# makezur/super_primitive

Hardware: AMD Instinct MI355X
Metric: GN iters/sec (640x480x64-seg frame pairs) (higher is better)
Workload: dtype f32; 1 GPU; Replica-shaped two-frame SfM, 640x480, 64 segments (grid, 4 px overlap), pyramid level 0 of a 3-level pyramid; BASELINE.json configs[1]; pairs_per_gpu=384, segment_pixels_per_pair=373056, optimiser=gn, tile_points=8192, span_points=4096, granule=64

## Files before the change

### super_primitive_amd/csrc/sp_cost.hip

```cpp
#include <type_traits>

#include "sp_solve_device.h"

namespace {

struct TileCtx {
    gptr_u32 pix;
    gptr_f4 src4;
    gptr_f32 trg;
    Cam Ks;
    Warp w;
    float shift;
    float gain, bias;
    float ax, ay;
    uint32_t row_bytes;
    int Wl, Hl;
    int start, count;
};

struct Geo {
    float qx, qy, qz;
    float zinv, zi;
    float px, py, pz;
};
// ... 251 lines not shown
    f32x2 wxy; float m;
    f32x2 srg; float sb;
    uint32_t off0;
};

__device__ __forceinline__ void prepare2_at(const PairConsts& k, f32x2 colrow, bool src_ok, float d, const f32x4 s, Pending2& p);

template <bool DT = false>
__device__ __forceinline__ void prepare2(const TileCtx& c, const PairConsts& k, float shift, uint32_t pw, const f32x4 s, Pending2& p) {
    const f32x2 colrow{(float)(pw & 0xffffu), (float)((pw >> 16) & 0x7fffu)};
    const bool src_ok = (int32_t)pw < 0;
    const float d = DT ? s.w * shift : fast_exp(s.w + shift);
    prepare2_at(k, colrow, src_ok, d, s, p);
}

typedef const SpRunDesc __attribute__((address_space(4)))* cptr_rd;
__device__ __forceinline__ SpRunDesc rd_load(cptr_rd p) {
    SpRunDesc r;
    r.valid[0] = p->valid[0]; r.valid[1] = p->valid[1];
    r.d[0] = p->d[0]; r.d[1] = p->d[1];
    r.base[0] = p->base[0]; r.base[1] = p->base[1];
    r.k = p->k; r.runs = p->runs;
    return r;
}
__device__ __forceinline__ f32x2 rd_colrow(const SpRunDesc& r, f32x2 lane2) {
    const float step = __builtin_amdgcn_fmed3f(lane2.x + r.k, 0.f, 1.f);
    return pfma(step, f32x2{r.d[0], r.d[1]}, lane2) + f32x2{r.base[0], r.base[1]};
}
__device__ __forceinline__ float rd_depth(const SpRunDesc& r, float d) {
    const uint64_t m = ((uint64_t)r.valid[1] << 32) | r.valid[0];
    float o;
    asm("v_cndmask_b32_e64 %0, 0, %1, %2" : "=v"(o) : "v"(d), "s"(m));
    return o;
}
template <bool DT>
__device__ __forceinline__ void prepare2_rd(const PairConsts& k, float shift, const SpRunDesc& r, f32x2 lane2, const f32x4 s, Pending2& p) {
    const f32x2 colrow = rd_colrow(r, lane2);
    const float d = rd_depth(r, DT ? s.w * shift : fast_exp(s.w + shift));
    prepare2_at(k, colrow, true, d, s, p);
}
template <bool DT>
__device__ __forceinline__ void prepare_rd(const TileCtx& c, float shift, float ifx, float ify, const SpRunDesc& r, f32x2 lane2, const f32x4 s,
                                           Pending& p) {
    const f32x2 colrow = rd_colrow(r, lane2);
    const float d = rd_depth(r, DT ? s.w * shift : fast_exp(s.w + shift));
    float x, y;
    backproject(colrow.x, colrow.y, d, c.Ks, ifx, ify, x, y);
    prepare_xyz(c, x, y, d, true, s.x, s.y, s.z, p);
}

__device__ __forceinline__ void prepare2_at(const PairConsts& k, f32x2 colrow, bool src_ok, float d, const f32x4 s, Pending2& p) {
    const f32x2 xy = pfma(colrow, k.ifxy, k.nKc) * d;
    const f32x2 qxy = pfma(k.R03, f32x2{xy.x, xy.x}, pfma(k.R14, f32x2{xy.y, xy.y}, pfma(k.R25, f32x2{d, d}, k.t01)));
    const float qz = fmaf(k.R6, xy.x, fmaf(k.R7, xy.y, fmaf(k.R8, d, k.t2)));
    const bool zguard = fabsf(qz) > 1e-6f;
    const float zinv = zguard ? __builtin_amdgcn_rcpf(qz) : 1e-6f;
    const f32x2 uv = qxy * k.Kf * zinv + k.Ktc;
    const f32x2 n = pfma(uv, k.invWH, f32x2{-1.f, -1.f});
    const bool ok = (fabsf(n.x) <= 0.99f) && (fabsf(n.y) <= 0.99f) && (qz > k.zmin) && src_ok && (d > 1e-7f);
    p.m = ok ? 1.f : 0.f;
    p.qxy = qxy; p.qz = qz;
    p.zinv = ok ? zinv : 0.f;
    p.zi = (ok && zguard) ? zinv : 0.f;
    p.srg = f32x2{s.x, s.y}; p.sb = s.z;
    const f32x2 ixy = pfma(n, k.sxy, k.sxy);
    const f32x2 fl{floorf(ixy.x), floorf(ixy.y)};
    p.wxy = ixy - fl;
    p.off0 = (uint32_t)fmaf(fl.y, k.row_bytes_f, fl.x * (float)(4u * SP_TEXEL_FLOATS));
}

struct Mix2 { f32x2 wa, wb, v; };
struct MixA { f32x2 ua, ub; };
// ... 141 lines not shown
    k.shift = cursor_shift<DT>(k.nq_kld, k.nq_kpl);
    cursor_fetch_next<TRIP>(k);
    return true;
}

template <bool WT>
__device__ __forceinline__ void store_partial(float* p, float v) {
    if (WT) __hip_atomic_store(p, v, __ATOMIC_RELAXED, __HIP_MEMORY_SCOPE_AGENT);
    else *p = v;
}

__device__ __forceinline__ int lane_id() { return (int)__builtin_amdgcn_mbcnt_hi(~0u, __builtin_amdgcn_mbcnt_lo(~0u, 0u)); }

template <bool WT, bool AFF = false>
__device__ __forceinline__ void flush_segment_gn(GnAcc& A, float* __restrict__ rec, AffAcc* aa = nullptr) {
    const int lane = lane_id();
    int pos; bool ok;
    if constexpr (AFF) {
        float v[10] = {A.hd01.x, A.hd01.y, A.hd[0].x, A.hd[0].y, A.hd[1].x, A.hd[1].y, A.D.x + A.D.y, A.bd.x + A.bd.y, aa->hda, aa->hdb};
        wave_sum_to_lanes<10>(v, lane, pos, ok);
        if (ok) store_partial<WT>(rec + pos, v[0]);
        aa->hda = 0.f; aa->hdb = 0.f;
    } else {
        float v[10] = {A.hd01.x, A.hd01.y, A.hd[0].x, A.hd[0].y, A.hd[1].x, A.hd[1].y, A.D.x + A.D.y, A.bd.x + A.bd.y,
                       A.cost - A.cost_mark, A.n - A.n_mark};
        wave_sum_to_lanes<10>(v, lane, pos, ok);
        if (ok) store_partial<WT>(rec + pos, v[0]);
        A.cost_mark = A.cost; A.n_mark = A.n;
    }
    const f32x2 z{0.f, 0.f};
    A.hd01 = z; A.hd[0] = z; A.hd[1] = z; A.D = z; A.bd = z;
}

template <bool DT, bool WT, bool AFF = false, bool W64 = false, bool RD = false>
__device__ __forceinline__ void run_span_gn(const TileCtx& c, const SpPair& pr, const int4* __restrict__ chunks, int q0,
                                            int n_chunks, int total, float irls_eps, float* __restrict__ span_rec,
                                            float* __restrict__ seg_partials, float* lds, const SpRunDesc* rd = nullptr) {
    static_assert(!RD || (W64 && DT && !AFF), "run descriptors: wave spans on depth tables");
    constexpr int TRIP = W64 ? 64 : SP_BLOCK;
    constexpr int NV = AFF ? SP_GNA_PARTIAL_FLOATS : SP_GN_PARTIAL_FLOATS, NS = AFF ? SP_GNA_SEG_FLOATS : SP_GN_SEG_FLOATS;
    GnAcc A;
    AffAcc AA;
    MixA ma{f32x2{0.f, 0.f}, f32x2{0.f, 0.f}};
    {
        const f32x2 z{0.f, 0.f};
        AA.haa = AA.hab = AA.hbb = AA.ba = AA.bb = AA.hda = AA.hdb = 0.f;
        AA.pa01 = z; AA.pb01 = z; AA.pa[0] = z; AA.pa[1] = z; AA.pb[0] = z; AA.pb[1] = z;
    }
    {
        const f32x2 z{0.f, 0.f};
        A.h00 = z; A.bp01 = z; A.hd01 = z;
#pragma unroll
        for (int k = 0; k < 2; ++k) { A.h0[k] = z; A.h1[k] = z; A.bp[k] = z; A.hd[k] = z; }
#pragma unroll
        for (int k = 0; k < 6; ++k) A.blk[k] = z;
        A.D = z; A.bd = z;
        A.h11 = A.cost = A.n = A.cost_mark = A.n_mark = 0.f;
    }
    const int wave = __builtin_amdgcn_readfirstlane((int)(threadIdx.x >> 6));
    SpanCursor k;
    cursor_init<TRIP, DT>(k, pr, chunks, q0, n_chunks);
    const int start = k.chunks[q0].start;
    PairConsts kc;
    {
        const Warp& w = c.w;
        kc.ifxy = sgpr2(1.f / c.Ks.fx, 1.f / c.Ks.fy);
        kc.nKc = f32x2{-c.Ks.cx * (1.f / c.Ks.fx), -c.Ks.cy * (1.f / c.Ks.fy)};
        kc.R03 = sgpr2(w.R[0], w.R[3]);        kc.R14 = sgpr2(w.R[1], w.R[4]);      kc.R25 = sgpr2(w.R[2], w.R[5]);
        kc.t01 = f32x2{w.t[0], w.t[1]};        kc.Kf = sgpr2(w.Kt.fx, w.Kt.fy);     kc.Ktc = sgpr2(w.Kt.cx, w.Kt.cy);
        kc.invWH = sgpr2(2.f * w.invWm1, 2.f * w.invHm1);  kc.sxy = sgpr2(w.sx, w.sy);
        kc.gab = sgpr2(c.gain * c.ax * w.Kt.fx, c.gain * c.ay * w.Kt.fy);
        kc.bias2 = f32x2{c.bias, c.bias};      kc.eps2 = sgpr2(irls_eps, irls_eps);
        kc.R6 = sgpr(w.R[6]); kc.R7 = sgpr(w.R[7]); kc.R8 = sgpr(w.R[8]); kc.t2 = w.t[2];
        asm volatile("" : "+v"(kc.nKc), "+v"(kc.bias2), "+v"(kc.t01), "+v"(kc.t2));
        kc.gain = sgpr(c.gain); kc.bias = sgpr(c.bias); kc.zmin = sgpr(w.zmin); kc.eps = sgpr(irls_eps);
        kc.row_bytes_f = sgpr((float)(c.Wl * (int)(4u * SP_TEXEL_FLOATS)));
    }
    const rsrc_t r_pix = make_rsrc(c.pix + start, (uint32_t)total * 4u);
    const rsrc_t r_src = make_rsrc(c.src4 + start, (uint32_t)total * 16u);
    const rsrc_t r_trg = make_rsrc(c.trg, (uint32_t)c.Wl * (uint32_t)c.Hl * (4u * SP_TEXEL_FLOATS));
    const int n_iter = total / TRIP;
    uint32_t op = (W64 ? (threadIdx.x & 63u) : threadIdx.x) * 4u;
    constexpr int NT = 2;
    cptr_rd rg = (cptr_rd)rd + (start >> 6);
    f32x2 lane2{(float)(threadIdx.x & 63u), 0.f};
    if (RD) asm volatile("" : "+v"(lane2));
    struct Slot { Pending2 p; int q; bool last; };
    Slot S0, S1;
    {
        const f32x4 s = buf_load4<NT>(r_src, op * 4u);
        if (RD) prepare2_rd<DT>(kc, k.shift, rd_load(rg), lane2, s, S0.p);
        else {
            const uint32_t pw = (uint32_t)__builtin_amdgcn_raw_buffer_load_b32(r_pix, (int)op, 0, NT);
            prepare2<DT>(c, kc, k.shift, pw, s, S0.p);
        }
        S0.last = cursor_advance<TRIP, DT>(k, S0.q);
    }
    S1.p = S0.p;
    S1.p.zinv = 0.f; S1.p.zi = 0.f;
    S1.q = q0; S1.last = false;
    Mix2 m{f32x2{0.f, 0.f}, f32x2{0.f, 0.f}, f32x2{0.f, 0.f}};
    auto trip = [&](Slot& a, Slot& b) {
        op += 4u * TRIP;
        asm volatile("" : "+v"(op));
        const uint32_t pw = RD ? 0u : (uint32_t)__builtin_amdgcn_raw_buffer_load_b32(r_pix, (int)op, 0, NT);
        const f32x4 s = buf_load4<NT>(r_src, op * 4u);
        SpRunDesc rn;
        if (RD) { ++rg; rn = rd_load(rg); }
        f32x3 ta = buf_load3(r_trg, a.p.off0);
        f32x3 tb = buf_load3(r_trg, a.p.off0 + 4u * SP_TEXEL_FLOATS);
        f32x3 tc = buf_load3(r_trg, a.p.off0, c.row_bytes);
        f32x3 td = buf_load3(r_trg, a.p.off0 + 4u * SP_TEXEL_FLOATS, c.row_bytes);
        __builtin_amdgcn_sched_barrier(0);
        fold_gn2<AFF>(kc, GeoGn{b.p.qxy, b.p.qz, b.p.zinv, b.p.zi}, m, A, &ma, &AA);
        if (b.last) flush_segment_gn<WT, AFF>(A, seg_partials + (size_t)(W64 ? b.q : 4 * b.q + wave) * NS, &AA);
        __builtin_amdgcn_sched_barrier(0);
        asm volatile("" : "+v"(ta), "+v"(tb), "+v"(tc), "+v"(td), "+v"(A.blk[0]), "+v"(A.blk[1]), "+v"(A.blk[2]),
                     "+v"(A.blk[3]), "+v"(A.blk[4]), "+v"(A.blk[5]), "+v"(A.bp[0]), "+v"(A.bp[1]), "+v"(A.hd[0]),
                     "+v"(A.hd[1]), "+v"(A.D), "+v"(A.bd), "+v"(A.h00), "+v"(A.h0[0]), "+v"(A.h0[1]), "+v"(A.h1[0]), "+v"(A.h1[1]), "+v"(A.h11), "+v"(A.bp01), "+v"(A.hd01));
        finish_gn2<AFF>(kc, a.p, ta, tb, tc, td, m, A.cost, A.n, &ma, &AA);
        uint32_t pw_ = pw;
        f32x4 s_ = s;
        if (RD) asm volatile("" : "+v"(s_));
        else asm volatile("" : "+v"(pw_), "+v"(s_));
        if (RD) prepare2_rd<DT>(kc, k.shift, rn, lane2, s_, b.p);
        else prepare2<DT>(c, kc, k.shift, pw_, s_, b.p);
        b.last = cursor_advance<TRIP, DT>(k, b.q);
    };
    int j = 0;
    for (; j + 1 < n_iter; j += 2) { trip(S0, S1); trip(S1, S0); }
    if (j < n_iter) {
        trip(S0, S1);
        fold_gn2<AFF>(kc, GeoGn{S0.p.qxy, S0.p.qz, S0.p.zinv, S0.p.zi}, m, A, &ma, &AA);
        flush_segment_gn<WT, AFF>(A, seg_partials + (size_t)(W64 ? S0.q : 4 * S0.q + wave) * NS, &AA);
    } else {
        fold_gn2<AFF>(kc, GeoGn{S1.p.qxy, S1.p.qz, S1.p.zinv, S1.p.zi}, m, A, &ma, &AA);
        flush_segment_gn<WT, AFF>(A, seg_partials + (size_t)(W64 ? S1.q : 4 * S1.q + wave) * NS, &AA);
    }
    float acc[NV];
    acc[0] = A.cost;
    acc[1] = A.h00.x; acc[2] = A.h00.y;
    acc[3] = A.h0[0].x; acc[4] = A.h0[0].y; acc[5] = A.h0[1].x; acc[6] = A.h0[1].y;
    acc[7] = A.h11;
    acc[8] = A.h1[0].x; acc[9] = A.h1[0].y; acc[10] = A.h1[1].x; acc[11] = A.h1[1].y;
    acc[12] = A.blk[0].x; acc[13] = A.blk[0].y; acc[14] = A.blk[1].x; acc[15] = A.blk[1].y;
    acc[16] = A.blk[2].y; acc[17] = A.blk[3].x; acc[18] = A.blk[3].y;
    acc[19] = A.blk[4].x; acc[20] = A.blk[4].y; acc[21] = A.blk[5].y;
    acc[22] = A.bp01.x; acc[23] = A.bp01.y;
    acc[24] = A.bp[0].x; acc[25] = A.bp[0].y; acc[26] = A.bp[1].x; acc[27] = A.bp[1].y;
    acc[28] = A.n;
    if constexpr (AFF) {
        acc[29] = AA.haa; acc[30] = AA.hab; acc[31] = AA.hbb; acc[32] = AA.ba; acc[33] = AA.bb;
        acc[34] = AA.pa01.x; acc[35] = AA.pa01.y; acc[36] = AA.pa[0].x; acc[37] = AA.pa[0].y; acc[38] = AA.pa[1].x; acc[39] = AA.pa[1].y;
        acc[40] = AA.pb01.x; acc[41] = AA.pb01.y; acc[42] = AA.pb[0].x; acc[43] = AA.pb[0].y; acc[44] = AA.pb[1].x; acc[45] = AA.pb[1].y;
        acc[46] = acc[47] = 0.f;
    } else {
        acc[29] = acc[30] = acc[31] = 0.f;
    }
    if (W64) {
        int pos; bool ok;
        wave_sum_to_lanes<NV>(acc, (int)((op >> 2) & 63u), pos, ok);
        if (ok) store_partial<WT>(span_rec + pos, acc[0]);
    } else {
        const int tid = (int)((op >> 2) & (uint32_t)(SP_BLOCK - 1));
        const float tot = block_sum_to_thread<NV>(acc, lds, tid);
        if (tid < NV) store_partial<WT>(span_rec + tid, tot);
    }
}

template <bool DT, bool WT, bool W64 = false, bool RD = false>
__device__ __forceinline__ void run_span_grad(const TileCtx& c, const SpPair& pr, const int4* __restrict__ chunks, int q0,
                                              int n_chunks, int total, float* __restrict__ span_rec,
                                              float* __restrict__ seg_partials, float* lds, const SpRunDesc* rd = nullptr) {
    static_assert(!RD || (W64 && DT), "run descriptors: wave spans on depth tables");
    constexpr int TRIP = W64 ? 64 : SP_BLOCK;
    constexpr int NV = SP_GRAD_PARTIAL_FLOATS;
    float acc[NV];
#pragma unroll
    for (int i = 0; i < NV; ++i) acc[i] = 0.f;
    const int wave = __builtin_amdgcn_readfirstlane((int)(threadIdx.x >> 6));
    SpanCursor k;
    cursor_init<TRIP, DT>(k, pr, chunks, q0, n_chunks);
    const int start = k.chunks[q0].start;
    const float ifx = 1.f / c.Ks.fx, ify = 1.f / c.Ks.fy;
    const rsrc_t r_pix = make_rsrc(c.pix + start, (uint32_t)total * 4u);
    const rsrc_t r_src = make_rsrc(c.src4 + start, (uint32_t)total * 16u);
    const rsrc_t r_trg = make_rsrc(c.trg, (uint32_t)c.Wl * (uint32_t)c.Hl * (4u * SP_TEXEL_FLOATS));
    const int n_iter = total / TRIP;
    uint32_t op = (W64 ? (threadIdx.x & 63u) : threadIdx.x) * 4u;
    constexpr int NT = 2;
    cptr_rd rg = (cptr_rd)rd + (start >> 6);
    f32x2 lane2{(float)(threadIdx.x & 63u), 0.f};
    if (RD) asm volatile("" : "+v"(lane2));
    struct Slot { Pending p; int q; bool last; };
    Slot S0, S1;
    {
        const f32x4 s = buf_load4<NT>(r_src, op * 4u);
        if (RD) prepare_rd<DT>(c, k.shift, ifx, ify, rd_load(rg), lane2, s, S0.p);
        else {
            const uint32_t pw = (uint32_t)__builtin_amdgcn_raw_buffer_load_b32(r_pix, (int)op, 0, NT);
// ... 175 lines not shown
    int32_t first_block;
    uint32_t mask;
    int32_t vspans;
};
struct SchedCost {
    const SpPair* pairs[SP_MAX_PHASES];
    float irls_eps[SP_MAX_PHASES];
    uint32_t mask;
    int32_t vspans;
    int32_t n_lists;
    SchedList list[SP_SCHED_LISTS];
};
struct FuseArgs {
    int32_t* arrivals;
    AdamArgs adam;
    GnArgs gn;
    const int32_t* done;
    const int32_t* phase;
    SchedCost sched;
    const int32_t* active;
    const MultiList* multi;
    int32_t n_multi;
    const uint32_t* rd_pix;
    const SpRunDesc* rd_desc;
};

constexpr int FORM_LOG_DEPTH = 0, FORM_DEPTH = 6;

struct Pix;
struct RunDesc;
template <class SRC>
struct CostFrom {
template <int MODE, int FORM = FORM_LOG_DEPTH, int FUSED = 0, bool W64 = false>
static __global__ __launch_bounds__(SP_BLOCK, FUSED != 0 ? 1 : (MODE == 2 ? 2 : 4)) void k_cost_pairs(
        const SpPair* __restrict__ pairs, const int4* __restrict__ chunks, const int4* __restrict__ spans, int n_spans,
        float irls_eps, float* __restrict__ partials, float* __restrict__ seg_partials, FuseArgs f) {
    static_assert(FORM == FORM_LOG_DEPTH || FORM == FORM_DEPTH, "FORM: log-depth tables (0) or depth tables (6)");
    constexpr bool RD = std::is_same<SRC, RunDesc>::value;
    constexpr bool DT = FORM == FORM_DEPTH;
    constexpr int NV = MODE == 0 ? SP_GRAD_PARTIAL_FLOATS : (MODE == 2 ? SP_GNA_PARTIAL_FLOATS : SP_GN_PARTIAL_FLOATS);
    __shared__ float lds[SP_WAVES * NV];
    int block = blockIdx.x;
    uint32_t phase_mask = f.sched.mask;
    int vspans = f.sched.vspans;
    if (f.multi) {
        int l = 0;
        for (int i = 1; i < f.n_multi && block >= f.multi[i].first_block; ++i) l = i;
        const MultiList& ml = f.multi[l];
        block -= ml.first_block;
        pairs = ml.pairs; chunks = reinterpret_cast<const int4*>(ml.chunks); spans = reinterpret_cast<const int4*>(ml.spans);
        n_spans = ml.n_spans; partials = ml.partials; seg_partials = ml.seg_partials;
    }
    if (f.phase && f.sched.n_lists > 0) {
        int l = 0;
#pragma unroll
        for (int i = 1; i < SP_SCHED_LISTS; ++i)
            if (i < f.sched.n_lists && block >= f.sched.list[i].first_block) l = i;
        const SchedList& sl = f.sched.list[l];
        block -= sl.first_block;
        chunks = sl.chunks; spans = sl.spans; n_spans = sl.n_spans; partials = sl.partials; seg_partials = sl.seg_partials;
        phase_mask = sl.mask;
        vspans = sl.vspans;
    }
    int w = W64 ? 4 * xcd_chunked_tile(block, (n_spans + 3) >> 2) + __builtin_amdgcn_readfirstlane((int)(threadIdx.x >> 6))
                : xcd_chunked_tile(block, n_spans);
    if (w >= n_spans) return;
    int owner;
// ... 7 lines not shown
        pairs = f.sched.pairs[ph];
        irls_eps = f.sched.irls_eps[ph];
        if (j >= pairs[owner].n_tiles) return;
        w = pairs[owner].tile0 + j;
        span = spans[w];
    } else {
        span = spans[w];
        owner = span.w;
        if (f.done && f.done[owner]) return;
        if (f.phase) {
            const int ph = f.phase[owner];
            if (ph >= SP_MAX_PHASES || ph < 0 || !((phase_mask >> ph) & 1u)) return;
            pairs = f.sched.pairs[ph];
            irls_eps = f.sched.irls_eps[ph];
        }
    }
    const SpPair& pr = pairs[owner];
    TileCtx c;
    c.pix = (gptr_u32)pr.pix;
    c.src4 = (gptr_f4)pr.src4;
    c.trg = (gptr_f32)pr.trg3;
    c.Ks = Cam{pr.K_src[0], pr.K_src[1], pr.K_src[2], pr.K_src[3]};
    const Cam Kt{pr.K_trg[0], pr.K_trg[1], pr.K_trg[2], pr.K_trg[3]};
    fill_warp(c, pr.pose, Kt, pr.H, pr.W, pr.Hl, pr.Wl, pr.zmin);
    c.shift = 0.f;
    c.gain = 1.f; c.bias = 0.f;
    if (pr.aff) {
        c.gain = sgpr(expf(-(pr.aff[2] - pr.aff[0])));
        c.bias = sgpr(pr.aff[3] - pr.aff[1]);
    }
    c.start = 0; c.count = 0;
    const SpRunDesc* rd = RD ? f.rd_desc + ((const uint32_t*)pr.pix - f.rd_pix) / 64 : nullptr;
    if (MODE == 2) run_span_gn<DT, FUSED != 0, true>(c, pr, chunks, span.x, span.y, span.z, irls_eps, partials + (size_t)w * NV, seg_partials, lds);
    else if (MODE == 1) run_span_gn<DT, FUSED != 0, false, W64, RD>(c, pr, chunks, span.x, span.y, span.z, irls_eps, partials + (size_t)w * NV, seg_partials, lds, rd);
    else run_span_grad<DT, FUSED != 0, W64, RD>(c, pr, chunks, span.x, span.y, span.z, partials + (size_t)w * NV, seg_partials, lds, rd);
    if (FUSED != 0) {
        __shared__ int is_last;
        asm volatile("s_waitcnt vmcnt(0)" ::: "memory");
        __syncthreads();
        if (threadIdx.x == 0) {
            const int old = __hip_atomic_fetch_add(f.arrivals + span.w, 1, __ATOMIC_RELAXED, __HIP_MEMORY_SCOPE_AGENT);
            const int last = old == pr.n_tiles - 1;
            if (last) {
                __hip_atomic_store(f.arrivals + span.w, 0, __ATOMIC_RELAXED, __HIP_MEMORY_SCOPE_AGENT);
                __builtin_amdgcn_fence(__ATOMIC_ACQUIRE, "agent");
            }
            is_last = last;
        }
        __syncthreads();
        if (is_last) {
            if (FUSED == 1) solve_adam(pairs, span.w, partials, seg_partials, f.adam);
            else solve_gn(pairs, span.w, partials, seg_partials, f.gn);
        }
    }
}
};

struct CostVariant {
    int mode;
    bool dt, w64, rd;
    int fused;
};
using CostKernel = void (*)(const SpPair*, const int4*, const int4*, int, float, float*, float*, FuseArgs);
CostKernel cost_kernel(const CostVariant& v) {
    enum { DT = 4, W64 = 8, RD = 16, ADAM = 32, GN = 2 * ADAM };
    if (v.mode < 0 || v.mode > 2 || v.fused < 0 || v.fused > 2) return nullptr;
    switch (v.mode | (v.dt ? DT : 0) | (v.w64 ? W64 : 0) | (v.rd ? RD : 0) | v.fused * ADAM) {
// ... 305 lines not shown
```

Before: 443,100 iters/s.

## Process two pixel groups per lane with packed-math Gauss-Newton span kernel

Adds a new wave-span GN path that handles two 64-pixel groups per lane at once, packing their geometry, residuals and normal-equation accumulation into v_pk_* f32x2 instructions via inline asm. The goal is to raise packed-FMA throughput and expose more memory-level parallelism per wave. It also lowers the occupancy hint for that kernel variant to 2 blocks, since the doubled accumulators raise register pressure. The older W64/run-descriptor code in run_span_gn is removed and routed to the new function instead.

```diff
diff --git a/super_primitive_amd/csrc/sp_cost.hip b/super_primitive_amd/csrc/sp_cost.hip
--- a/super_primitive_amd/csrc/sp_cost.hip
+++ b/super_primitive_amd/csrc/sp_cost.hip
@@ -307,12 +307,6 @@
     float o;
     asm("v_cndmask_b32_e64 %0, 0, %1, %2" : "=v"(o) : "v"(d), "s"(m));
     return o;
-}
-template <bool DT>
-__device__ __forceinline__ void prepare2_rd(const PairConsts& k, float shift, const SpRunDesc& r, f32x2 lane2, const f32x4 s, Pending2& p) {
-    const f32x2 colrow = rd_colrow(r, lane2);
-    const float d = rd_depth(r, DT ? s.w * shift : fast_exp(s.w + shift));
-    prepare2_at(k, colrow, true, d, s, p);
 }
 template <bool DT>
 __device__ __forceinline__ void prepare_rd(const TileCtx& c, float shift, float ifx, float ify, const SpRunDesc& r, f32x2 lane2, const f32x4 s,
@@ -520,12 +514,444 @@
     A.hd01 = z; A.hd[0] = z; A.hd[1] = z; A.D = z; A.bd = z;
 }
 
-template <bool DT, bool WT, bool AFF = false, bool W64 = false, bool RD = false>
+typedef f32x2 P2;
+__device__ __forceinline__ P2 bc(float v) { return P2{v, v}; }
+__device__ __forceinline__ P2 lo2(P2 v) { return P2{v.x, v.x}; }
+__device__ __forceinline__ P2 hi2(P2 v) { return P2{v.y, v.y}; }
+
+struct PendingP {
+    P2 qx, qy, qz, zinv, zi;
+    P2 wx, wy, m;
+    f32x2 srgA, srgB;
+    P2 sb;
+    uint32_t offA, offB;
+};
+struct MixP { P2 w00, w01, w11, v0, v1, t; };
+struct AccP {
+    P2 h00, h01, h11, h0[4], h1[4];
+    P2 blk[10];
+    P2 bp[6];
+    P2 seg[10];
+    float cost, n;
+};
+
+__device__ __forceinline__ P2 psub2_lo(P2 a, f32x2 b) {
+    P2 d;
+    asm("v_pk_add_f32 %0, %1, %2 op_sel_hi:[1,0] neg_lo:[0,1] neg_hi:[0,1]" : "=v"(d) : "v"(a), "v"(b));
+    return d;
+}
+__device__ __forceinline__ P2 psub2_hi(P2 a, f32x2 b) {
+    P2 d;
+    asm("v_pk_add_f32 %0, %1, %2 op_sel:[0,1] op_sel_hi:[1,1] neg_lo:[0,1] neg_hi:[0,1]" : "=v"(d) : "v"(a), "v"(b));
+    return d;
+}
+__device__ __forceinline__ float fma3(float a, float b, float c) {
+    float d;
+    asm("v_fma_f32 %0, %1, %2, %3" : "=v"(d) : "v"(a), "v"(b), "v"(c));
+    return d;
+}
+__device__ __forceinline__ P2 pfma_s_lo(f32x2 s, P2 b, f32x2 c) {
+    P2 d;
+    asm("v_pk_fma_f32 %0, %1, %2, %3 op_sel_hi:[0,1,0]" : "=v"(d) : "s"(s), "v"(b), "v"(c));
+    return d;
+}
+__device__ __forceinline__ P2 pfma_s_hi(f32x2 s, P2 b, f32x2 c) {
+    P2 d;
+    asm("v_pk_fma_f32 %0, %1, %2, %3 op_sel:[1,0,1] op_sel_hi:[1,1,1]" : "=v"(d) : "s"(s), "v"(b), "v"(c));
+    return d;
+}
+__device__ __forceinline__ P2 pmul_b_lo(P2 a, f32x2 B) {
+    P2 d;
+    asm("v_pk_mul_f32 %0, %1, %2 op_sel_hi:[1,0]" : "=v"(d) : "v"(a), "v"(B));
+    return d;
+}
+__device__ __forceinline__ P2 pmul_b_hi(P2 a, f32x2 B) {
+    P2 d;
+    asm("v_pk_mul_f32 %0, %1, %2 op_sel:[0,1] op_sel_hi:[1,1]" : "=v"(d) : "v"(a), "v"(B));
+    return d;
+}
+__device__ __forceinline__ P2 pfma_c_lo(P2 a, P2 b, f32x2 C) {
+    P2 d;
+    asm("v_pk_fma_f32 %0, %1, %2, %3 op_sel_hi:[1,1,0]" : "=v"(d) : "v"(a), "v"(b), "v"(C));
+    return d;
+}
+__device__ __forceinline__ P2 pfma_c_hi(P2 a, P2 b, f32x2 C) {
+    P2 d;
+    asm("v_pk_fma_f32 %0, %1, %2, %3 op_sel:[0,0,1] op_sel_hi:[1,1,1]" : "=v"(d) : "v"(a), "v"(b), "v"(C));
+    return d;
+}
+__device__ __forceinline__ P2 pfma_bc_lo(P2 a, f32x2 B, f32x2 C) {
+    P2 d;
+    asm("v_pk_fma_f32 %0, %1, %2, %3 op_sel_hi:[1,0,0]" : "=v"(d) : "v"(a), "v"(B), "v"(C));
+    return d;
+}
+__device__ __forceinline__ P2 pfma_bc_hi(P2 a, f32x2 B, f32x2 C) {
+    P2 d;
+    asm("v_pk_fma_f32 %0, %1, %2, %3 op_sel:[0,1,1] op_sel_hi:[1,1,1]" : "=v"(d) : "v"(a), "v"(B), "v"(C));
+    return d;
+}
+__device__ __forceinline__ P2 pfma_b_m1_lo(P2 a, f32x2 B) {
+    P2 d;
+    asm("v_pk_fma_f32 %0, %1, %2, -1.0 op_sel_hi:[1,0,0]" : "=v"(d) : "v"(a), "v"(B));
+    return d;
+}
+__device__ __forceinline__ P2 pfma_b_m1_hi(P2 a, f32x2 B) {
+    P2 d;
+    asm("v_pk_fma_f32 %0, %1, %2, -1.0 op_sel:[0,1,0] op_sel_hi:[1,1,0]" : "=v"(d) : "v"(a), "v"(B));
+    return d;
+}
+__device__ __forceinline__ P2 pfma_b_lo(P2 a, f32x2 B, P2 c) {
+    P2 d;
+    asm("v_pk_fma_f32 %0, %1, %2, %3 op_sel_hi:[1,0,1]" : "=v"(d) : "v"(a), "v"(B), "v"(c));
+    return d;
+}
+__device__ __forceinline__ P2 pfma_b_hi(P2 a, f32x2 B, P2 c) {
+    P2 d;
+    asm("v_pk_fma_f32 %0, %1, %2, %3 op_sel:[0,1,0] op_sel_hi:[1,1,1]" : "=v"(d) : "v"(a), "v"(B), "v"(c));
+    return d;
+}
+__device__ __forceinline__ P2 pfma_xy(P2 a, f32x2 B) {
+    P2 d;
+    asm("v_pk_fma_f32 %0, %1, %2, %2 op_sel:[0,0,1] op_sel_hi:[1,0,1]" : "=v"(d) : "v"(a), "v"(B));
+    return d;
+}
+__device__ __forceinline__ bool all5(bool a, bool b, bool c, bool d, bool e) {
+    return ((int)a & (int)b & (int)c & (int)d & (int)e) != 0;
+}
+__device__ __forceinline__ float absmax_s(float r, float eps) {
+    float m;
+    asm("v_max_f32 %0, |%1|, %2" : "=v"(m) : "v"(r), "s"(eps));
+    return m;
+}
+
+struct RunDescP { float kA, kB; P2 d0, d1, b0, b1; uint64_t validA, validB; };
+__device__ __forceinline__ RunDescP rd_load_pp(cptr_rd a, cptr_rd b) {
+    RunDescP r;
+    r.kA = a->k; r.kB = b->k;
+    r.d0 = P2{a->d[0], b->d[0]}; r.d1 = P2{a->d[1], b->d[1]};
+    r.b0 = P2{a->base[0], b->base[0]}; r.b1 = P2{a->base[1], b->base[1]};
+    r.validA = ((uint64_t)a->valid[1] << 32) | a->valid[0];
+    r.validB = ((uint64_t)b->valid[1] << 32) | b->valid[0];
+    return r;
+}
+__device__ __forceinline__ float rd_step(float lane, float k) {
+    float o;
+    asm("v_add_f32_e64 %0, %1, %2 clamp" : "=v"(o) : "v"(lane), "s"(k));
+    return o;
+}
+
+struct PairConstsP {
+    f32x2 R03, R14, R25;
+    float zmin, eps, row_bytes_f;
+    f32x2 ifxy, nKc, t01, Kf, Ktc, invWH, sxy, gab, R67, R8t2, gain_bias;
+};
+__device__ __forceinline__ PairConstsP pair_consts_pp(const TileCtx& c, float irls_eps) {
+    PairConstsP k;
+    const Warp& w = c.w;
+    k.R03 = sgpr2(w.R[0], w.R[3]); k.R14 = sgpr2(w.R[1], w.R[4]); k.R25 = sgpr2(w.R[2], w.R[5]);
+    k.zmin = sgpr(w.zmin); k.eps = sgpr(irls_eps);
+    k.row_bytes_f = sgpr((float)(c.Wl * (int)(4u * SP_TEXEL_FLOATS)));
+    k.ifxy = f32x2{1.f / c.Ks.fx, 1.f / c.Ks.fy};
+    k.nKc = f32x2{-c.Ks.cx * (1.f / c.Ks.fx), -c.Ks.cy * (1.f / c.Ks.fy)};
+    k.t01 = f32x2{w.t[0], w.t[1]};
+    k.Kf = f32x2{w.Kt.fx, w.Kt.fy}; k.Ktc = f32x2{w.Kt.cx, w.Kt.cy};
+    k.invWH = f32x2{2.f * w.invWm1, 2.f * w.invHm1};
+    k.sxy = f32x2{w.sx, w.sy};
+    k.gab = f32x2{c.gain * c.ax * w.Kt.fx, c.gain * c.ay * w.Kt.fy};
+    k.R67 = f32x2{w.R[6], w.R[7]}; k.R8t2 = f32x2{w.R[8], w.t[2]};
+    k.gain_bias = f32x2{c.gain, c.bias};
+    asm volatile("" : "+v"(k.ifxy), "+v"(k.nKc), "+v"(k.t01), "+v"(k.Kf), "+v"(k.Ktc), "+v"(k.invWH), "+v"(k.sxy), "+v"(k.gab), "+v"(k.R67),
+                 "+v"(k.R8t2), "+v"(k.gain_bias));
+    return k;
+}
+
+template <bool DT, bool RD>
+__device__ __forceinline__ void prepare_pp(const PairConstsP& k, float sh_lo, float sh_hi, uint32_t pwA, uint32_t pwB, const RunDescP& r,
+                                           P2 lane2, const f32x4 sA, const f32x4 sB, PendingP& p) {
+    P2 col, row;
+    P2 d = DT ? P2{sA.w * sh_lo, sB.w * sh_hi} : P2{fast_exp(sA.w + sh_lo), fast_exp(sB.w + sh_hi)};
+    bool srcA = true, srcB = true;
+    if constexpr (RD) {
+        const P2 step{rd_step(lane2.x, r.kA), rd_step(lane2.x, r.kB)};
+        const P2 c0 = pfma(step, r.d0, lane2);
+        col = c0 + r.b0;
+        const P2 r0 = step * r.d1;
+        row = r0 + r.b1;
+        srcA = __builtin_amdgcn_inverse_ballot_w64(r.validA); srcB = __builtin_amdgcn_inverse_ballot_w64(r.validB);
+    } else {
+        col = P2{(float)(pwA & 0xffffu), (float)(pwB & 0xffffu)};
+        row = P2{(float)((pwA >> 16) & 0x7fffu), (float)((pwB >> 16) & 0x7fffu)};
+        srcA = (int32_t)pwA < 0; srcB = (int32_t)pwB < 0;
+    }
+    const P2 x = pfma_bc_lo(col, k.ifxy, k.nKc) * d;
+    const P2 y = pfma_bc_hi(row, k.ifxy, k.nKc) * d;
+    const P2 qx = pfma(lo2(k.R03), x, pfma(lo2(k.R14), y, pfma_s_lo(k.R25, d, k.t01)));
+    const P2 qy = pfma(hi2(k.R03), x, pfma(hi2(k.R14), y, pfma_s_hi(k.R25, d, k.t01)));
+    const P2 qz = pfma_b_lo(x, k.R67, pfma_b_hi(y, k.R67, pfma_xy(d, k.R8t2)));
+    const bool zgA = fabsf(qz.x) > 1e-6f, zgB = fabsf(qz.y) > 1e-6f;
+    const P2 zinv{zgA ? __builtin_amdgcn_rcpf(qz.x) : 1e-6f, zgB ? __builtin_amdgcn_rcpf(qz.y) : 1e-6f};
+    const P2 fxq = pmul_b_lo(qx, k.Kf), fyq = pmul_b_hi(qy, k.Kf);
+    const P2 u = pfma_c_lo(fxq, zinv, k.Ktc), v = pfma_c_hi(fyq, zinv, k.Ktc);
+    const P2 nx = pfma_b_m1_lo(u, k.invWH), ny = pfma_b_m1_hi(v, k.invWH);
+    const bool okA = all5(fabsf(nx.x) <= 0.99f, fabsf(ny.x) <= 0.99f, qz.x > k.zmin, srcA, d.x > 1e-7f);
+    const bool okB = all5(fabsf(nx.y) <= 0.99f, fabsf(ny.y) <= 0.99f, qz.y > k.zmin, srcB, d.y > 1e-7f);
+    p.m = P2{okA ? 1.f : 0.f, okB ? 1.f : 0.f};
+    p.qx = qx; p.qy = qy; p.qz = qz;
+    p.zinv = P2{okA ? zinv.x : 0.f, okB ? zinv.y : 0.f};
+    p.zi = P2{(okA & zgA) ? zinv.x : 0.f, (okB & zgB) ? zinv.y : 0.f};
+    p.srgA = f32x2{sA.x, sA.y}; p.srgB = f32x2{sB.x, sB.y}; p.sb = P2{sA.z, sB.z};
+    const P2 ix = pfma_bc_lo(nx, k.sxy, k.sxy), iy = pfma_bc_hi(ny, k.sxy, k.sxy);
+    const P2 flx{floorf(ix.x), floorf(ix.y)}, fly{floorf(iy.x), floorf(iy.y)};
+    p.wx = psub2(ix, flx);
+    p.wy = psub2(iy, fly);
+    const P2 off = pfma(fly, bc(k.row_bytes_f), flx * bc((float)(4u * SP_TEXEL_FLOATS)));
+    p.offA = (uint32_t)off.x; p.offB = (uint32_t)off.y;
+}
+
+__device__ __forceinline__ void finish_pp(const PairConstsP& k, const PendingP& p, const f32x3 aA, const f32x3 bA, const f32x3 cA,
+                                          const f32x3 dA, const f32x3 aB, const f32x3 bB, const f32x3 cB, const f32x3 dB, MixP& o) {
+    struct Ch { P2 Gx, Gy, r; };
+    auto rg = [&](const f32x3 a, const f32x3 b, const f32x3 c, const f32x3 d, P2 wx, P2 wy, f32x2 src) {
+        const P2 a2{a.x, a.y}, b2{b.x, b.y}, c2{c.x, c.y}, d2{d.x, d.y};
+        const P2 e1 = psub2(b2, a2), e2 = psub2(c2, a2), e3 = psub2(psub2(d2, c2), e1);
+        Ch ch;
+        ch.Gy = pfma(wx, e3, e2);
+        ch.Gx = pfma(wy, e3, e1);
+        const P2 it = pfma(wy, ch.Gy, pfma(wx, e1, a2));
+        ch.r = psub2(src, pfma_xy(it, k.gain_bias));
+        return ch;
+    };
+    const Ch cA_ = rg(aA, bA, cA, dA, lo2(p.wx), lo2(p.wy), p.srgA);
+    const Ch cB_ = rg(aB, bB, cB, dB, hi2(p.wx), hi2(p.wy), p.srgB);
+    Ch cb;
+    {
+        const P2 e1{bA.z - aA.z, bB.z - aB.z}, e2{cA.z - aA.z, cB.z - aB.z}, t{dA.z - cA.z, dB.z - cB.z};
+        const P2 e3 = psub2(t, e1);
+        cb.Gy = pfma(p.wx, e3, e2);
+        cb.Gx = pfma(p.wy, e3, e1);
+        const P2 it = pfma(p.wy, cb.Gy, P2{fma3(p.wx.x, e1.x, aA.z), fma3(p.wx.y, e1.y, aB.z)});
+        cb.r = psub2(p.sb, pfma_xy(it, k.gain_bias));
+    }
+    auto wgt = [&](P2 r) { return P2{__builtin_amdgcn_rcpf(absmax_s(r.x, k.eps)), __builtin_amdgcn_rcpf(absmax_s(r.y, k.eps))}; };
+    const P2 wA = wgt(cA_.r), wB = wgt(cB_.r), wb = wgt(cb.r);
+    const P2 wGxA = wA * cA_.Gx, wGyA = wA * cA_.Gy, wGxB = wB * cB_.Gx, wGyB = wB * cB_.Gy, wGxb = wb * cb.Gx, wGyb = wb * cb.Gy;
+    auto dot = [&](P2 xA, P2 yA, P2 xB, P2 yB, P2 xb, P2 yb) {
+        P2 s = xb * yb;
+        s.x = fmaf(xA.y, yA.y, fmaf(xA.x, yA.x, s.x));
+        s.y = fmaf(xB.y, yB.y, fmaf(xB.x, yB.x, s.y));
+        return s;
+    };
+    o.w00 = dot(wGxA, cA_.Gx, wGxB, cB_.Gx, wGxb, cb.Gx);
+    o.w01 = dot(wGxA, cA_.Gy, wGxB, cB_.Gy, wGxb, cb.Gy);
+    o.w11 = dot(wGyA, cA_.Gy, wGyB, cB_.Gy, wGyb, cb.Gy);
+    o.v0 = dot(wGxA, cA_.r, wGxB, cB_.r, wGxb, cb.r);
+    o.v1 = dot(wGyA, cA_.r, wGyB, cB_.r, wGyb, cb.r);
+    o.t = P2{(fabsf(cA_.r.x) + fabsf(cA_.r.y)) + fabsf(cb.r.x), (fabsf(cB_.r.x) + fabsf(cB_.r.y)) + fabsf(cb.r.y)};
+}
+
+__device__ __forceinline__ void fold_pp(const PairConstsP& k, const PendingP& g, const MixP& w, AccP& A) {
+    const P2 ga = pmul_b_lo(g.zinv, k.gab), gb = pmul_b_hi(g.zinv, k.gab);
+    const P2 W00 = w.w00 * (ga * ga), W01 = w.w01 * (ga * gb), W11 = w.w11 * (gb * gb);
+    const P2 V0 = -(w.v0 * ga), V1 = -(w.v1 * gb);
+    const P2 ux = g.qx * g.zi, vy = g.qy * g.zi;
+    const P2 ez = psub2_hi(g.qz, k.R8t2);
+    const P2 Q0 = pfma(-ez, ux, psub2_lo(g.qx, k.t01)), Q1 = pfma(-ez, vy, psub2_hi(g.qy, k.t01));
+    const P2 n02 = ux, n03 = ux * g.qy, a04 = pfma(ux, g.qx, g.qz), n05 = g.qy;
+    const P2 n12 = vy, n13 = pfma(vy, g.qy, g.qz), a14 = vy * g.qx, a15 = g.qx;
+    const P2 nB02 = pfma(W00, n02, W01 * n12), nB03 = pfma(W00, n03, W01 * n13), B04 = pfma(W00, a04, W01 * a14), B05 = pfma(-W00, n05, W01 * a15);
+    const P2 nB12 = pfma(W01, n02, W11 * n12), nB13 = pfma(W01, n03, W11 * n13), B14 = pfma(W01, a04, W11 * a14), B15 = pfma(-W01, n05, W11 * a15);
+    const P2 P0 = pfma(Q0, W00, Q1 * W01), P1 = pfma(Q0, W01, Q1 * W11);
+    A.h00 += W00; A.h01 += W01; A.h11 += W11;
+    A.h0[0] = psub2(A.h0[0], nB02); A.h0[1] = psub2(A.h0[1], nB03); A.h0[2] += B04; A.h0[3] += B05;
+    A.h1[0] = psub2(A.h1[0], nB12); A.h1[1] = psub2(A.h1[1], nB13); A.h1[2] += B14; A.h1[3] += B15;
+    A.blk[0] = pfma(n02, nB02, pfma(n12, nB12, A.blk[0]));
+    A.blk[1] = pfma(n02, nB03, pfma(n12, nB13, A.blk[1]));
+    A.blk[2] = pfma(-n02, B04, pfma(-n12, B14, A.blk[2]));
+    A.blk[3] = pfma(-n02, B05, pfma(-n12, B15, A.blk[3]));
+    A.blk[4] = pfma(n03, nB03, pfma(n13, nB13, A.blk[4]));
+    A.blk[5] = pfma(-n03, B04, pfma(-n13, B14, A.blk[5]));
+    A.blk[6] = pfma(-n03, B05, pfma(-n13, B15, A.blk[6]));
+    A.blk[7] = pfma(a04, B04, pfma(a14, B14, A.blk[7]));
+    A.blk[8] = pfma(a04, B05, pfma(a14, B15, A.blk[8]));
+    A.blk[9] = pfma(-n05, B05, pfma(a15, B15, A.blk[9]));
+    A.bp[0] += V0; A.bp[1] += V1;
+    A.bp[2] = pfma(-V0, n02, pfma(-V1, n12, A.bp[2]));
+    A.bp[3] = pfma(-V0, n03, pfma(-V1, n13, A.bp[3]));
+    A.bp[4] = pfma(V0, a04, pfma(V1, a14, A.bp[4]));
+    A.bp[5] = pfma(-V0, n05, pfma(V1, a15, A.bp[5]));
+    A.seg[0] += P0; A.seg[1] += P1;
+    A.seg[2] = pfma(-P0, n02, pfma(-P1, n12, A.seg[2]));
+    A.seg[3] = pfma(-P0, n03, pfma(-P1, n13, A.seg[3]));
+    A.seg[4] = pfma(P0, a04, pfma(P1, a14, A.seg[4]));
+    A.seg[5] = pfma(-P0, n05, pfma(P1, a15, A.seg[5]));
+    A.seg[6] = pfma(Q0, P0, pfma(Q1, P1, A.seg[6]));
+    A.seg[7] = pfma(Q0, V0, pfma(Q1, V1, A.seg[7]));
+    A.seg[8] = pfma(g.m, w.t, A.seg[8]);
+    A.seg[9] += g.m;
+}
+
+template <bool WT, bool ALL>
+__device__ __forceinline__ void flush_segment_pp(AccP& A, float* __restrict__ rec) {
+    float v[10];
+#pragma unroll
+    for (int i = 0; i < 10; ++i) {
+        v[i] = ALL ? A.seg[i].x + A.seg[i].y : A.seg[i].x;
+        A.seg[i] = ALL ? P2{0.f, 0.f} : P2{0.f, A.seg[i].y};
+    }
+    A.cost += v[8]; A.n += v[9];
+    int pos; bool ok;
+    wave_sum_to_lanes<10>(v, lane_id(), pos, ok);
+    if (ok) store_partial<WT>(rec + pos, v[0]);
+}
+
+template <bool DT>
+__device__ __forceinline__ int cursor_advance_pp(SpanCursor& k, const SpPair& pr) {
+    if (--k.left > 0) return 0;
+    ++k.q;
+    k.left = k.nq_left;
+    k.shift = sgpr(cursor_shift<DT>(k.nq_kld, k.nq_kpl));
+    asm volatile("" : "+s"(k.shift));
+    if (k.q + 1 < k.q_end) {
+        const SpPair* p = &pr;
+        asm volatile("" : "+s"(p));
+        const int seg = k.chunks[k.q + 1].seg;
+        k.nq_left = k.chunks[k.q + 1].count / 64;
+        k.nq_kld = ((cptr_f32)p->kld)[seg];
+        k.nq_kpl = ((cptr_f32)p->kp_L)[seg];
+    }
+    return 1;
+}
+
+template <bool DT, bool WT, bool RD>
+__device__ __forceinline__ void run_span_gn_pp(const TileCtx& c, const SpPair& pr, const int4* __restrict__ chunks, int q0, int n_chunks,
+                                               int total, float irls_eps, float* __restrict__ span_rec, float* __restrict__ seg_partials,
+                                               const SpRunDesc* rd) {
+    static_assert(!RD || DT, "run descriptors: depth tables");
+    constexpr int NV = SP_GN_PARTIAL_FLOATS, NS = SP_GN_SEG_FLOATS;
+    AccP A;
+    {
+        const P2 z{0.f, 0.f};
+        A.h00 = z; A.h01 = z; A.h11 = z;
+#pragma unroll
+        for (int i = 0; i < 4; ++i) { A.h0[i] = z; A.h1[i] = z; }
+#pragma unroll
+        for (int i = 0; i < 10; ++i) { A.blk[i] = z; A.seg[i] = z; }
+#pragma unroll
+        for (int i = 0; i < 6; ++i) A.bp[i] = z;
+        A.cost = A.n = 0.f;
+    }
+    SpanCursor k;
+    cursor_init<64, DT>(k, pr, chunks, q0, n_chunks);
+    k.shift = sgpr(k.shift);
+    const int start = k.chunks[q0].start;
+    const PairConstsP kc = pair_consts_pp(c, irls_eps);
+    const rsrc_t r_pix = make_rsrc(c.pix + start, (uint32_t)total * 4u);
+    const rsrc_t r_src = make_rsrc(c.src4 + start, (uint32_t)total * 16u);
+    const rsrc_t r_trg = make_rsrc(c.trg, (uint32_t)c.Wl * (uint32_t)c.Hl * (4u * SP_TEXEL_FLOATS));
+    const int n_groups = total / 64;
+    const int g_end = (n_groups + 1) & ~1;
+    uint32_t op = (threadIdx.x & 63u) * 4u;
+    constexpr int NT = 2;
+    const cptr_rd rg0 = (cptr_rd)rd + (start >> 6);
+    int g = 0;
+    P2 lane2 = bc((float)(threadIdx.x & 63u));
+    if (RD) asm volatile("" : "+v"(lane2));
+    struct Slot { PendingP p; int q, last; };
+    Slot S0, S1;
+    auto prepare = [&](uint32_t pwA, uint32_t pwB, const RunDescP& r, const f32x4 sA, const f32x4 sB, Slot& s) {
+        const float sh_lo = k.shift;
+        s.q = k.q;
+        s.last = cursor_advance_pp<DT>(k, pr);
+        const float sh_hi = k.shift;
+        s.last |= (cursor_advance_pp<DT>(k, pr) & (int)(g + 1 < n_groups)) << 1;
+        prepare_pp<DT, RD>(kc, sh_lo, sh_hi, pwA, pwB, r, lane2, sA, sB, s.p);
+        g += 2;
+    };
+    auto rd_next = [&]() {
+        RunDescP r{};
+        if constexpr (RD) r = rd_load_pp(rg0 + min(g, n_groups), rg0 + min(g + 1, n_groups));
+        return r;
+    };
+    {
+        const f32x4 sA = buf_load4<NT>(r_src, op * 4u), sB = buf_load4<NT>(r_src, op * 4u + 64u * 16u);
+        const uint32_t pwA = RD ? 0u : (uint32_t)__builtin_amdgcn_raw_buffer_load_b32(r_pix, (int)op, 0, NT);
+        const uint32_t pwB = RD ? 0u : (uint32_t)__builtin_amdgcn_raw_buffer_load_b32(r_pix, (int)(op + 64u * 4u), 0, NT);
+        prepare(pwA, pwB, rd_next(), sA, sB, S0);
+    }
+    S1.p = S0.p;
+    S1.p.zinv = S1.p.zi = S1.p.m = P2{0.f, 0.f};
+    S1.q = q0; S1.last = 0;
+    MixP m;
+    m.w00 = m.w01 = m.w11 = m.v0 = m.v1 = m.t = P2{0.f, 0.f};
+    auto fold = [&](Slot& b) {
+        if (b.last & 1) {
+#pragma unroll
+            for (int i = 0; i < 10; ++i) A.seg[i] = P2{A.seg[i].x + A.seg[i].y, 0.f};
+        }
+        fold_pp(kc, b.p, m, A);
+        if (b.last) {
+            if (b.last & 1) flush_segment_pp<WT, false>(A, seg_partials + (size_t)b.q * NS);
+            if (b.last & 2) flush_segment_pp<WT, true>(A, seg_partials + (size_t)(b.q + (b.last & 1)) * NS);
+        }
+    };
+    auto trip = [&](Slot& a, Slot& b) {
+        op += 4u * 128u;
+        asm volatile("" : "+v"(op));
+        const uint32_t pwA = RD ? 0u : (uint32_t)__builtin_amdgcn_raw_buffer_load_b32(r_pix, (int)op, 0, NT);
+        const uint32_t pwB = RD ? 0u : (uint32_t)__builtin_amdgcn_raw_buffer_load_b32(r_pix, (int)(op + 64u * 4u), 0, NT);
+        const f32x4 sA = buf_load4<NT>(r_src, op * 4u), sB = buf_load4<NT>(r_src, op * 4u + 64u * 16u);
+        const RunDescP rn = rd_next();
+        constexpr uint32_t TX = 4u * SP_TEXEL_FLOATS;
+        f32x3 aA = buf_load3(r_trg, a.p.offA), bA = buf_load3(r_trg, a.p.offA + TX);
+        f32x3 cA = buf_load3(r_trg, a.p.offA, c.row_bytes), dA = buf_load3(r_trg, a.p.offA + TX, c.row_bytes);
+        f32x3 aB = buf_load3(r_trg, a.p.offB), bB = buf_load3(r_trg, a.p.offB + TX);
+        f32x3 cB = buf_load3(r_trg, a.p.offB, c.row_bytes), dB = buf_load3(r_trg, a.p.offB + TX, c.row_bytes);
+        __builtin_amdgcn_sched_barrier(0);
+        fold(b);
+        __builtin_amdgcn_sched_barrier(0);
+        asm volatile("" : "+v"(aA), "+v"(bA), "+v"(cA), "+v"(dA), "+v"(aB), "+v"(bB), "+v"(cB), "+v"(dB), "+v"(A.h00), "+v"(A.h01), "+v"(A.h11),
+                     "+v"(A.h0[0]), "+v"(A.h0[1]), "+v"(A.h0[2]), "+v"(A.h0[3]), "+v"(A.h1[0]), "+v"(A.h1[1]), "+v"(A.h1[2]), "+v"(A.h1[3]));
+        asm volatile("" : "+v"(A.blk[0]), "+v"(A.blk[1]), "+v"(A.blk[2]), "+v"(A.blk[3]), "+v"(A.blk[4]), "+v"(A.blk[5]), "+v"(A.blk[6]),
+                     "+v"(A.blk[7]), "+v"(A.blk[8]), "+v"(A.blk[9]), "+v"(A.bp[0]), "+v"(A.bp[1]), "+v"(A.bp[2]), "+v"(A.bp[3]), "+v"(A.bp[4]),
+                     "+v"(A.bp[5]));
+        asm volatile("" : "+v"(A.seg[0]), "+v"(A.seg[1]), "+v"(A.seg[2]), "+v"(A.seg[3]), "+v"(A.seg[4]), "+v"(A.seg[5]), "+v"(A.seg[6]),
+                     "+v"(A.seg[7]), "+v"(A.seg[8]), "+v"(A.seg[9]));
+        finish_pp(kc, a.p, aA, bA, cA, dA, aB, bB, cB, dB, m);
+        asm volatile("" : "+v"(m.w00), "+v"(m.w01), "+v"(m.w11), "+v"(m.v0), "+v"(m.v1), "+v"(m.t));
+        uint32_t pwA_ = pwA, pwB_ = pwB;
+        f32x4 sA_ = sA, sB_ = sB;
+        if (RD) asm volatile("" : "+v"(sA_), "+v"(sB_));
+        else asm volatile("" : "+v"(pwA_), "+v"(pwB_), "+v"(sA_), "+v"(sB_));
+        prepare(pwA_, pwB_, rn, sA_, sB_, b);
+    };
+    while (g < g_end) { trip(S0, S1); trip(S1, S0); }
+    if (g == g_end) {
+        trip(S0, S1);
+        fold(S0);
+    } else {
+        fold(S1);
+    }
+    float acc[NV];
+    acc[0] = A.cost;
+    acc[1] = A.h00.x + A.h00.y; acc[2] = A.h01.x + A.h01.y; acc[7] = A.h11.x + A.h11.y;
+#pragma unroll
+    for (int i = 0; i < 4; ++i) { acc[3 + i] = A.h0[i].x + A.h0[i].y; acc[8 + i] = A.h1[i].x + A.h1[i].y; }
+#pragma unroll
+    for (int i = 0; i < 10; ++i) acc[12 + i] = A.blk[i].x + A.blk[i].y;
+#pragma unroll
+    for (int i = 0; i < 6; ++i) acc[22 + i] = A.bp[i].x + A.bp[i].y;
+    acc[28] = A.n;
+    acc[29] = acc[30] = acc[31] = 0.f;
+    int pos; bool ok;
+    wave_sum_to_lanes<NV>(acc, (int)((op >> 2) & 63u), pos, ok);
+    if (ok) store_partial<WT>(span_rec + pos, acc[0]);
+}
+
+template <bool DT, bool WT, bool AFF = false>
 __device__ __forceinline__ void run_span_gn(const TileCtx& c, const SpPair& pr, const int4* __restrict__ chunks, int q0,
                                             int n_chunks, int total, float irls_eps, float* __restrict__ span_rec,
-                                            float* __restrict__ seg_partials, float* lds, const SpRunDesc* rd = nullptr) {
-    static_assert(!RD || (W64 && DT && !AFF), "run descriptors: wave spans on depth tables");
-    constexpr int TRIP = W64 ? 64 : SP_BLOCK;
+                                            float* __restrict__ seg_partials, float* lds) {
+    constexpr int TRIP = SP_BLOCK;
     constexpr int NV = AFF ? SP_GNA_PARTIAL_FLOATS : SP_GN_PARTIAL_FLOATS, NS = AFF ? SP_GNA_SEG_FLOATS : SP_GN_SEG_FLOATS;
     GnAcc A;
     AffAcc AA;
@@ -568,20 +994,14 @@
     const rsrc_t r_src = make_rsrc(c.src4 + start, (uint32_t)total * 16u);
     const rsrc_t r_trg = make_rsrc(c.trg, (uint32_t)c.Wl * (uint32_t)c.Hl * (4u * SP_TEXEL_FLOATS));
     const int n_iter = total / TRIP;
-    uint32_t op = (W64 ? (threadIdx.x & 63u) : threadIdx.x) * 4u;
+    uint32_t op = threadIdx.x * 4u;
     constexpr int NT = 2;
-    cptr_rd rg = (cptr_rd)rd + (start >> 6);
-    f32x2 lane2{(float)(threadIdx.x & 63u), 0.f};
-    if (RD) asm volatile("" : "+v"(lane2));
     struct Slot { Pending2 p; int q; bool last; };
     Slot S0, S1;
     {
         const f32x4 s = buf_load4<NT>(r_src, op * 4u);
-        if (RD) prepare2_rd<DT>(kc, k.shift, rd_load(rg), lane2, s, S0.p);
-        else {
-            const uint32_t pw = (uint32_t)__builtin_amdgcn_raw_buffer_load_b32(r_pix, (int)op, 0, NT);
-            prepare2<DT>(c, kc, k.shift, pw, s, S0.p);
-        }
+        const uint32_t pw = (uint32_t)__builtin_amdgcn_raw_buffer_load_b32(r_pix, (int)op, 0, NT);
+        prepare2<DT>(c, kc, k.shift, pw, s, S0.p);
         S0.last = cursor_advance<TRIP, DT>(k, S0.q);
     }
     S1.p = S0.p;
@@ -591,17 +1011,15 @@
     auto trip = [&](Slot& a, Slot& b) {
         op += 4u * TRIP;
         asm volatile("" : "+v"(op));
-        const uint32_t pw = RD ? 0u : (uint32_t)__builtin_amdgcn_raw_buffer_load_b32(r_pix, (int)op, 0, NT);
+        const uint32_t pw = (uint32_t)__builtin_amdgcn_raw_buffer_load_b32(r_pix, (int)op, 0, NT);
         const f32x4 s = buf_load4<NT>(r_src, op * 4u);
-        SpRunDesc rn;
-        if (RD) { ++rg; rn = rd_load(rg); }
         f32x3 ta = buf_load3(r_trg, a.p.off0);
         f32x3 tb = buf_load3(r_trg, a.p.off0 + 4u * SP_TEXEL_FLOATS);
         f32x3 tc = buf_load3(r_trg, a.p.off0, c.row_bytes);
         f32x3 td = buf_load3(r_trg, a.p.off0 + 4u * SP_TEXEL_FLOATS, c.row_bytes);
         __builtin_amdgcn_sched_barrier(0);
         fold_gn2<AFF>(kc, GeoGn{b.p.qxy, b.p.qz, b.p.zinv, b.p.zi}, m, A, &ma, &AA);
-        if (b.last) flush_segment_gn<WT, AFF>(A, seg_partials + (size_t)(W64 ? b.q : 4 * b.q + wave) * NS, &AA);
+        if (b.last) flush_segment_gn<WT, AFF>(A, seg_partials + (size_t)(4 * b.q + wave) * NS, &AA);
         __builtin_amdgcn_sched_barrier(0);
         asm volatile("" : "+v"(ta), "+v"(tb), "+v"(tc), "+v"(td), "+v"(A.blk[0]), "+v"(A.blk[1]), "+v"(A.blk[2]),
                      "+v"(A.blk[3]), "+v"(A.blk[4]), "+v"(A.blk[5]), "+v"(A.bp[0]), "+v"(A.bp[1]), "+v"(A.hd[0]),
@@ -609,10 +1027,8 @@
         finish_gn2<AFF>(kc, a.p, ta, tb, tc, td, m, A.cost, A.n, &ma, &AA);
         uint32_t pw_ = pw;
         f32x4 s_ = s;
-        if (RD) asm volatile("" : "+v"(s_));
-        else asm volatile("" : "+v"(pw_), "+v"(s_));
-        if (RD) prepare2_rd<DT>(kc, k.shift, rn, lane2, s_, b.p);
-        else prepare2<DT>(c, kc, k.shift, pw_, s_, b.p);
+        asm volatile("" : "+v"(pw_), "+v"(s_));
+        prepare2<DT>(c, kc, k.shift, pw_, s_, b.p);
         b.last = cursor_advance<TRIP, DT>(k, b.q);
     };
     int j = 0;
@@ -620,10 +1036,10 @@
     if (j < n_iter) {
         trip(S0, S1);
         fold_gn2<AFF>(kc, GeoGn{S0.p.qxy, S0.p.qz, S0.p.zinv, S0.p.zi}, m, A, &ma, &AA);
-        flush_segment_gn<WT, AFF>(A, seg_partials + (size_t)(W64 ? S0.q : 4 * S0.q + wave) * NS, &AA);
+        flush_segment_gn<WT, AFF>(A, seg_partials + (size_t)(4 * S0.q + wave) * NS, &AA);
     } else {
         fold_gn2<AFF>(kc, GeoGn{S1.p.qxy, S1.p.qz, S1.p.zinv, S1.p.zi}, m, A, &ma, &AA);
-        flush_segment_gn<WT, AFF>(A, seg_partials + (size_t)(W64 ? S1.q : 4 * S1.q + wave) * NS, &AA);
+        flush_segment_gn<WT, AFF>(A, seg_partials + (size_t)(4 * S1.q + wave) * NS, &AA);
     }
     float acc[NV];
     acc[0] = A.cost;
@@ -645,15 +1061,9 @@
     } else {
         acc[29] = acc[30] = acc[31] = 0.f;
     }
-    if (W64) {
-        int pos; bool ok;
-        wave_sum_to_lanes<NV>(acc, (int)((op >> 2) & 63u), pos, ok);
-        if (ok) store_partial<WT>(span_rec + pos, acc[0]);
-    } else {
-        const int tid = (int)((op >> 2) & (uint32_t)(SP_BLOCK - 1));
-        const float tot = block_sum_to_thread<NV>(acc, lds, tid);
-        if (tid < NV) store_partial<WT>(span_rec + tid, tot);
-    }
+    const int tid = (int)((op >> 2) & (uint32_t)(SP_BLOCK - 1));
+    const float tot = block_sum_to_thread<NV>(acc, lds, tid);
+    if (tid < NV) store_partial<WT>(span_rec + tid, tot);
 }
 
 template <bool DT, bool WT, bool W64 = false, bool RD = false>
@@ -895,7 +1305,7 @@
 template <class SRC>
 struct CostFrom {
 template <int MODE, int FORM = FORM_LOG_DEPTH, int FUSED = 0, bool W64 = false>
-static __global__ __launch_bounds__(SP_BLOCK, FUSED != 0 ? 1 : (MODE == 2 ? 2 : 4)) void k_cost_pairs(
+static __global__ __launch_bounds__(SP_BLOCK, FUSED != 0 ? 1 : (MODE == 2 || (MODE == 1 && W64) ? 2 : 4)) void k_cost_pairs(
         const SpPair* __restrict__ pairs, const int4* __restrict__ chunks, const int4* __restrict__ spans, int n_spans,
         float irls_eps, float* __restrict__ partials, float* __restrict__ seg_partials, FuseArgs f) {
     static_assert(FORM == FORM_LOG_DEPTH || FORM == FORM_DEPTH, "FORM: log-depth tables (0) or depth tables (6)");
@@ -969,7 +1379,8 @@
     c.start = 0; c.count = 0;
     const SpRunDesc* rd = RD ? f.rd_desc + ((const uint32_t*)pr.pix - f.rd_pix) / 64 : nullptr;
     if (MODE == 2) run_span_gn<DT, FUSED != 0, true>(c, pr, chunks, span.x, span.y, span.z, irls_eps, partials + (size_t)w * NV, seg_partials, lds);
-    else if (MODE == 1) run_span_gn<DT, FUSED != 0, false, W64, RD>(c, pr, chunks, span.x, span.y, span.z, irls_eps, partials + (size_t)w * NV, seg_partials, lds, rd);
+    else if (MODE == 1 && W64) run_span_gn_pp<DT, FUSED != 0, RD>(c, pr, chunks, span.x, span.y, span.z, irls_eps, partials + (size_t)w * NV, seg_partials, rd);
+    else if (MODE == 1) run_span_gn<DT, FUSED != 0>(c, pr, chunks, span.x, span.y, span.z, irls_eps, partials + (size_t)w * NV, seg_partials, lds);
     else run_span_grad<DT, FUSED != 0, W64, RD>(c, pr, chunks, span.x, span.y, span.z, partials + (size_t)w * NV, seg_partials, lds, rd);
     if (FUSED != 0) {
         __shared__ int is_last;
```

Result: slower. 435,800 iters/s (-1.7%).
